# morrislab/rnascan

Measured on AMD Instinct MI355X. Metric: scored windows/sec (seq+struct, w=12), higher is better.
Workload: dtype f64

## Files before the change

include/pfmscan.h:

```cpp
#ifndef PFMSCAN_H
#define PFMSCAN_H

#include <stdint.h>

#ifdef __cplusplus
extern "C" {
#endif

#define PFMSCAN_ABI_VERSION 8
#define PFMSCAN_NCODE   8
#define PFMSCAN_SEP     7
#define PFMSCAN_NSTRUCT 7
#define PFMSCAN_MAX_M   64
#define PFMSCAN_MAX_WIDTH 4096

#define PFMSCAN_OK          0
#define PFMSCAN_E_BADARG   -1
#define PFMSCAN_E_BADSHAPE -2
#define PFMSCAN_E_OOM      -3
#define PFMSCAN_E_HIP      -4
#define PFMSCAN_E_CAPACITY -5

#define PFMSCAN_PROFILE_NONE 0
#define PFMSCAN_PROFILE_F32  1
// ... 138 lines not shown
                                     double *d_hit_struct, uint64_t *d_hit_count, void *stream);
int pfmscan_library_hits_letters_host(pfmscan_ctx *ctx, pfmscan_library *lib,
                                      const uint8_t *codes, const uint8_t *codes2, int64_t n_pos,
                                      const double *thr_seq, const double *thr_struct, int64_t capacity,
                                      int64_t *hit_pos, int32_t *hit_motif, float *hit_seq,
                                      double *hit_struct, int64_t *n_hits);

int pfmscan_debug_credit_table(const double *letter_table, int m, double thr_seq, int bits,
                               uint16_t *credits, double *slack);

int pfmscan_debug_quad_table(const double *letter_table, int m, double thr_seq, uint16_t *credits, double *slack);
int pfmscan_debug_library8_credits(const double *letter_table, int m, double thr, uint16_t *credits, double *slack);

int pfmscan_debug_credit8_table(const double *letter_table, int m, double thr, uint16_t *credits, int *mode);

#define PFMSCAN_UPLOAD_RUNTIME 0
#define PFMSCAN_UPLOAD_STAGED  1
int pfmscan_set_upload_mode(pfmscan_ctx *ctx, int mode);
int pfmscan_upload_source_file(pfmscan_ctx *ctx, const void *base, size_t length, const char *path, int64_t file_offset);
int pfmscan_upload_source_file_checked(pfmscan_ctx *ctx, const void *base, size_t length, const char *path,
                                       int64_t file_offset, int64_t st_dev, int64_t st_ino, int64_t st_size);

int pfmscan_count_bytes(const uint8_t *buf, int64_t n, int64_t *counts , int n_threads);
int pfmscan_fasta_lone_cr(const uint8_t *buf, int64_t n, int *found, int n_threads);
int pfmscan_fasta_index(const uint8_t *buf, int64_t n, int64_t capacity, int64_t *hdr_off,
                        int64_t *hdr_len, int64_t *seq_off, int64_t *seq_end, int64_t *n_letters,
                        int64_t *n_records, int n_threads);
int pfmscan_fasta_ids(const uint8_t *buf, const int64_t *hdr_off, const int64_t *hdr_len,
                      int64_t n_records, int64_t *id_off, int64_t *id_len, int *all_ascii);
int pfmscan_gather_spans(const uint8_t *buf, const int64_t *spans, int64_t n_spans, int separator,
// ... 52 lines not shown
```

rnascan_amd/_lib.py:

```python
import ctypes
import importlib.util
import os
import sys

import numpy as np

HERE = os.path.dirname(os.path.abspath(__file__))
LIB_PATH = os.environ.get("PFMSCAN_LIB") or os.path.join(HERE, "libpfmscan.so")

OK = 0
E_BADARG, E_BADSHAPE, E_OOM, E_HIP, E_CAPACITY = -1, -2, -3, -4, -5
PROFILE_NONE, PROFILE_F32, PROFILE_F64 = 0, 1, 2
SEP = 7
NCODE = 8
NSTRUCT = 7
MAX_M = 64
MAX_WIDTH = 4096
ABI_VERSION = 8

SYMBOLS = [
    "pfmscan_abi_version", "pfmscan_ctx_create", "pfmscan_ctx_destroy", "pfmscan_last_error",
    "pfmscan_device_info", "pfmscan_synchronize", "pfmscan_motif_create", "pfmscan_motif_destroy",
    "pfmscan_pwm_calculate", "pfmscan_scan_dev", "pfmscan_scan_letters_f64_dev", "pfmscan_hits_dev",
    "pfmscan_scan_host", "pfmscan_scan_letters_f64_host", "pfmscan_hits_host", "pfmscan_time_scan_dev",
    "pfmscan_stage", "pfmscan_scan_staged", "pfmscan_hits_staged", "pfmscan_hits_adaptive_dev",
    "pfmscan_library_create", "pfmscan_library_destroy", "pfmscan_library_info", "pfmscan_library_hits_dev",
    "pfmscan_library_hits_staged", "pfmscan_library_hits_host", "pfmscan_library_hits_pipeline_host", "pfmscan_debug_credit_table",
    "pfmscan_library_create_letters", "pfmscan_library_hits_letters_dev", "pfmscan_library_hits_letters_host", "pfmscan_debug_library8_credits",
    "pfmscan_debug_quad_table", "pfmscan_debug_credit8_table",
    "pfmscan_hits_pipeline_host", "pfmscan_staged_positions",
    "pfmscan_hits_letters_f64_dev", "pfmscan_hits_letters_f64_staged", "pfmscan_hits_letters_f64_host",
    "pfmscan_hits_pair_dev", "pfmscan_stage_codes2", "pfmscan_hits_pair_staged", "pfmscan_hits_pair_host", "pfmscan_round_decimals",
    "pfmscan_set_upload_mode", "pfmscan_upload_source_file", "pfmscan_upload_source_file_checked", "pfmscan_fasta_lone_cr", "pfmscan_count_bytes", "pfmscan_fasta_index", "pfmscan_fasta_ids", "pfmscan_gather_spans", "pfmscan_fasta_encode", "pfmscan_tsv_format", "pfmscan_profile_parse", "pfmscan_tsv_number",
    "pfmscan_place_alloc", "pfmscan_place_free", "pfmscan_place_note", "pfmscan_place_trim",
]
TSV_CONST, TSV_I64, TSV_F32, TSV_F64, TSV_INDEXED, TSV_FIXED, TSV_WINDOW, TSV_SPAN = range(8)


class TsvColumn(ctypes.Structure):
    _fields_ = [("kind", ctypes.c_int32), ("reserved", ctypes.c_int32), ("data", ctypes.c_void_p),
                ("aux", ctypes.c_void_p), ("blob", ctypes.c_void_p), ("width", ctypes.c_int64)]



# ... 60 lines not shown
    L.pfmscan_library_create_letters.argtypes = [vp, vp, vp, i32, i32, ctypes.POINTER(vp)]
    L.pfmscan_library_hits_letters_dev.argtypes = [vp, vp, vp, vp, i64, vp, vp, i64, vp, vp, vp, vp, vp, vp]
    L.pfmscan_library_hits_letters_host.argtypes = [vp, vp, vp, vp, i64, vp, vp, i64, vp, vp, vp, vp, ctypes.POINTER(i64)]
    L.pfmscan_library_destroy.argtypes = [vp]
    L.pfmscan_library_destroy.restype = None
    L.pfmscan_library_info.argtypes = [vp, ctypes.POINTER(i32), ctypes.POINTER(i32), ctypes.POINTER(i32), ctypes.POINTER(i32),
                                       ctypes.POINTER(dbl)]
    L.pfmscan_library_hits_dev.argtypes = [vp, vp, vp, vp, i32, i64, vp, vp, i64, vp, vp, vp, vp, vp, vp]
    L.pfmscan_library_hits_staged.argtypes = [vp, vp, vp, vp, i64, vp, vp, vp, vp, ctypes.POINTER(i64)]
    L.pfmscan_library_hits_host.argtypes = [vp, vp, vp, vp, i32, i64, vp, vp, i64, vp, vp, vp, vp, ctypes.POINTER(i64)]
    L.pfmscan_hits_pipeline_host.argtypes = [vp, vp, vp, vp, i32, i64, i64, dbl, dbl, i64, vp, vp, vp, ctypes.POINTER(i64)]
    L.pfmscan_library_hits_pipeline_host.argtypes = [vp, vp, vp, vp, i32, i64, i64, vp, vp, i64, vp, vp, vp, vp, ctypes.POINTER(i64)]
    L.pfmscan_debug_credit_table.argtypes = [vp, i32, dbl, i32, vp, ctypes.POINTER(dbl)]
    L.pfmscan_debug_quad_table.argtypes = [vp, i32, dbl, vp, ctypes.POINTER(dbl)]
    L.pfmscan_debug_credit8_table.argtypes = [vp, i32, dbl, vp, ctypes.POINTER(i32)]
    L.pfmscan_set_upload_mode.argtypes = [vp, i32]
    L.pfmscan_upload_source_file.argtypes = [vp, vp, ctypes.c_size_t, ctypes.c_char_p, i64]
    L.pfmscan_upload_source_file_checked.argtypes = [vp, vp, ctypes.c_size_t, ctypes.c_char_p, i64, i64, i64, i64]
    L.pfmscan_fasta_lone_cr.argtypes = [vp, i64, ctypes.POINTER(i32), i32]
    L.pfmscan_count_bytes.argtypes = [vp, i64, vp, i32]
    L.pfmscan_place_alloc.argtypes = [vp, i32, vp, vp, i32]
    L.pfmscan_place_free.argtypes = [vp, vp]
    L.pfmscan_place_trim.argtypes = [vp]
    L.pfmscan_place_note.argtypes = [vp]
    L.pfmscan_place_note.restype = ctypes.c_char_p
    L.pfmscan_fasta_index.argtypes = [vp, i64, i64, vp, vp, vp, vp, vp, ctypes.POINTER(i64), i32]
    L.pfmscan_fasta_ids.argtypes = [vp, vp, vp, i64, vp, vp, ctypes.POINTER(i32)]
    L.pfmscan_gather_spans.argtypes = [vp, vp, i64, i32, vp, i64, ctypes.POINTER(i64)]
    L.pfmscan_fasta_encode.argtypes = [vp, vp, vp, vp, i64, i64, vp, i32, vp, vp, i32]
    L.pfmscan_profile_parse.argtypes = [ctypes.c_char_p, i64, i32, i64, vp, ctypes.POINTER(i64)]
# ... 712 lines not shown
        if self.has_letters:
            ts = np.ascontiguousarray(np.broadcast_to(np.asarray(thr_seq, dtype=np.float64), (self.n,)))
        tt = None
        if self.has_struct:
            tt = np.ascontiguousarray(np.broadcast_to(np.asarray(-np.inf if thr_struct is None else thr_struct,
                                                                 dtype=np.float64), (self.n,)))
        return ts, tt

    def info(self):
        n, m, npass, per, eps = ctypes.c_int(), ctypes.c_int(), ctypes.c_int(), ctypes.c_int(), ctypes.c_double()
        self._ctx._check(self._L.pfmscan_library_info(self._h, ctypes.byref(n), ctypes.byref(m), ctypes.byref(npass),
                                                      ctypes.byref(per), ctypes.byref(eps)))
        return {"n_motifs": n.value, "m": m.value, "passes": npass.value, "motifs_per_pass": per.value,
                "max_prefilter_eps": eps.value}

    def close(self):
        if getattr(self, "_h", None) and getattr(self._ctx, "_h", None):
            self._L.pfmscan_library_destroy(self._h)
        self._h = None

    def __del__(self):
        try:
            self.close()
        except Exception:
            pass


def credit_table(letter_table, thr_seq, bits=16):
    L = load()
    T = np.ascontiguousarray(letter_table, dtype=np.float64)
    if T.ndim != 2 or T.shape[1] != NCODE:
        raise ValueError("letter_table must be [m][8]")
    m = T.shape[0]
    out = np.zeros(((m + 1) // 2, 16), dtype=np.uint16)
    slack = ctypes.c_double(0.0)
    rc = L.pfmscan_debug_credit_table(_ptr(T), m, float(thr_seq), int(bits), _ptr(out), ctypes.byref(slack))
    if rc != OK:
        raise ValueError("pfmscan_debug_credit_table: bad argument")
    return out, slack.value


def quad_table(letter_table, thr_seq):
    L = load()
    T = np.ascontiguousarray(letter_table, dtype=np.float64)
    if T.ndim != 2 or T.shape[1] != NCODE:
        raise ValueError("letter_table must be [m][8]")
    m = T.shape[0]
    out = np.zeros(((m + 3) // 4, 256), dtype=np.uint16)
    slack = ctypes.c_double(0.0)
    rc = L.pfmscan_debug_quad_table(_ptr(T), m, float(thr_seq), _ptr(out), ctypes.byref(slack))
    if rc != OK:
        raise ValueError("pfmscan_debug_quad_table: bad argument")
    return out, slack.value

# ... 55 lines not shown
```

rnascan_amd/build.py:

```python
import os
import re
import shutil
import subprocess
import sys
import tempfile
from concurrent.futures import ThreadPoolExecutor

HERE = os.path.dirname(os.path.abspath(__file__))
CSRC = os.path.join(HERE, "csrc")
OBJ = os.path.join(CSRC, "_obj")
LIB = os.path.join(HERE, "libpfmscan.so")
SOURCES = ["pfmscan_kernels.hip", "pfmscan_letters8.hip", "pfmscan_letters_fixed.hip", "pfmscan_api.hip", "pfmscan_sort.hip", "pfmscan_library.hip", "pfmscan_library_api.hip", "pfmscan_proflib.hip", "pfmscan_profile_fixed.hip", "pfmscan_place.hip",
           "pfmscan_pipeline.hip", "pfmscan_ingest.hip", "pfmscan_upload.hip"]
HEADERS = ["pfmscan_internal.hpp", "pfmscan_ctx.hpp", "pfmscan_device.hpp", "pfmscan_profile.hpp", "pfmscan_exact.hpp", os.path.join("..", "..", "include", "pfmscan.h")]
DEPS = SOURCES + HEADERS
FLAGS = ["-O3", "--offload-arch=gfx950", "-std=c++17", "-fPIC", "-fno-fast-math", "-Wall"]


def hipcc_path():
    for cand in (os.environ.get("HIPCC"), shutil.which("hipcc"), "/opt/rocm/bin/hipcc"):
        if cand and os.path.exists(cand):
            return cand
    raise RuntimeError("hipcc not found (set HIPCC or install ROCm under /opt/rocm)")


def stale():
    if not os.path.exists(LIB):
# ... 80 lines not shown
```

rnascan_amd/csrc/pfmscan_internal.hpp:

```cpp
#pragma once
#include <hip/hip_runtime.h>
#include <stdint.h>
#include <atomic>
#include "../../include/pfmscan.h"

namespace pfmscan {

struct CredCache {
    double thr = __builtin_nan("");
    int mode = 0;
    uint16_t cr[16 * 16];
};

struct Cred8Cache {
    double thr = __builtin_nan("");
    int mode = 0;
    uint16_t cr[32 * 8];
};

struct QuadSlot {
    double thr = __builtin_nan("");
    uint32_t *d_tab = nullptr;
    uint32_t *h_tab = nullptr;
    hipEvent_t ready = nullptr, used = nullptr;
// ... 169 lines not shown
    const void *profile;
    int profile_dtype;
    int64_t n_pos;
    const double *pssm;
    const double *thr;
    double struct_band;
    const int32_t *finite;
    int n_motifs, m, motif_base;
    int64_t pos_offset;
    int64_t shard_cap;
    int hit_shards;
    int64_t *hit_pos;
    int32_t *hit_motif;
    double *hit_struct;
    unsigned long long *hit_count;
};
hipError_t launch_profile_library(const ProfLibArgs &a, hipStream_t stream);
int64_t profile_library_tile();

hipError_t sort_temp_bytes(int64_t total, int key_bits, size_t *bytes);
hipError_t launch_gather_sorted(const GatherArgs &g, hipStream_t stream);

}
```

rnascan_amd/csrc/pfmscan_library_api.hip:

```cpp
#include <algorithm>
#include <cmath>
#include <cstdlib>
#include <cstring>
#include <new>
#include <string>
#include <vector>

#include "pfmscan_ctx.hpp"

using namespace pfmscan;

namespace {

struct LibPass {
    int motif_base = 0, n_real = 0, nmp = 0, ng = 0;
    int ng_real = 0;
    size_t pairs_off = 0;
    size_t letters_off = 0;
    size_t pssm_off = 0;
    size_t thr_off = 0;
};

}

// ... 56 lines not shown
                out[t * 16 + (c0 | c1 << 2)] = T[(2 * t) * 8 + c0] + (2 * t + 1 < m ? T[(2 * t + 1) * 8 + c1] : 0.0);
}

void pfmscan::quad_sums(const double *T, int m, double *out)
{
    const int nq = (m + 3) / 4;
    for (int t = 0; t < nq; ++t)
        for (int idx = 0; idx < 256; ++idx) {
            double v = 0.0;
            for (int i = 0; i < 4; ++i)
                if (4 * t + i < m) v += T[(4 * t + i) * 8 + ((idx >> (2 * i)) & 3)];
            out[t * 256 + idx] = v;
        }
}

struct pfmscan_library {
    pfmscan_ctx *ctx = nullptr;
    int n = 0, m = 0, npair = 0, np_bucket = 8;
    bool has_struct = false;
    bool has_letters = true;
    bool pair = false;
    bool letters8 = false;
    std::vector<double> rows8;
    double *d_pssm_rows = nullptr;
    int32_t *d_finite = nullptr;
    bool all_finite = false;
    double struct_band = 0.0;
    std::vector<double> pairsum;
    std::vector<LibPass> passes;
    uint16_t *d_pairs = nullptr;
    double *d_letters = nullptr, *d_pssm = nullptr, *d_thr = nullptr;
    size_t pairs_elems = 0, thr_elems = 0;
    std::vector<uint16_t> h_pairs;
    std::vector<double> h_thr;
    std::vector<double> cur_seq, cur_struct, eps;
    bool thr_valid = false;
};

static int lib_fail(pfmscan_ctx *ctx, int code, const std::string &msg) { return fail(ctx, code, msg); }

extern "C" {

// ... 18 lines not shown
        lib->has_struct = true;
        lib->has_letters = false;
        for (int k = 0; k < n_motifs; ++k) lib->struct_band = std::max(lib->struct_band, struct_band(struct_pssms + (size_t)k * m * 7, m));
        std::vector<int32_t> fin((size_t)n_motifs, 1);
        for (int k = 0; k < n_motifs; ++k)
            for (int i = 0; i < m * 7; ++i)
                if (!std::isfinite(struct_pssms[(size_t)k * m * 7 + i])) fin[(size_t)k] = 0;
        if (std::getenv("PFMSCAN_FORCE_GENERIC")) std::fill(fin.begin(), fin.end(), 0);
        const size_t cells = (size_t)n_motifs * m * 7;
        hipError_t e = hipMalloc((void **)&lib->d_pssm_rows, cells * 8);
        if (e == hipSuccess) e = hipMemcpy(lib->d_pssm_rows, struct_pssms, cells * 8, hipMemcpyHostToDevice);
        if (e == hipSuccess) e = hipMalloc((void **)&lib->d_finite, (size_t)n_motifs * 4);
        if (e == hipSuccess) e = hipMemcpy(lib->d_finite, fin.data(), (size_t)n_motifs * 4, hipMemcpyHostToDevice);
        if (e == hipSuccess) e = hipMalloc((void **)&lib->d_thr, (size_t)n_motifs * 8);
        lib->thr_elems = (size_t)n_motifs;
        if (e != hipSuccess) {
            pfmscan_library_destroy(lib);
            return fail_hip(ctx, e, "uploading the library tables");
        }
        *out = lib;
        return PFMSCAN_OK;
    }
    return create_seq_library(ctx, letter_tables, struct_pssms, 7, n_motifs, m, out);
}

}

static int create_seq_library(pfmscan_ctx *ctx, const double *letter_tables, const double *struct_pssms, int ncol, int n_motifs, int m,
                              pfmscan_library **out)
{
// ... 160 lines not shown
            return lib_fail(ctx, PFMSCAN_E_BADSHAPE, "column 7 of every letter table must be NaN (the foreign code)");
    if (seq_tables) return create_seq_library(ctx, seq_tables, struct_tables, 8, n_motifs, m, out);
    return create_letters8_library(ctx, struct_tables, n_motifs, m, out);
}

void pfmscan_library_destroy(pfmscan_library *lib)
{
    if (!lib) return;
    if (lib->ctx) (void)hipSetDevice(lib->ctx->device);
    if (lib->d_pairs) (void)hipFree(lib->d_pairs);
    if (lib->d_letters) (void)hipFree(lib->d_letters);
    if (lib->d_pssm) (void)hipFree(lib->d_pssm);
    if (lib->d_thr) (void)hipFree(lib->d_thr);
    if (lib->d_pssm_rows) (void)hipFree(lib->d_pssm_rows);
    if (lib->d_finite) (void)hipFree(lib->d_finite);
    delete lib;
}

int pfmscan_debug_credit_table(const double *letter_table, int m, double thr_seq, int bits, uint16_t *credits, double *slack)
{
    if (!letter_table || !credits || m < 1 || m > PFMSCAN_MAX_M || std::isnan(thr_seq)) return PFMSCAN_E_BADARG;
    if (bits == 0) bits = lib_credit_bits(lib_np_bucket(m));
    if (bits != 10 && bits != 16) return PFMSCAN_E_BADARG;
    const int npair = (m + 1) / 2;
    std::vector<double> ps((size_t)npair * 16);
    pair_sums(letter_table, m, ps.data());
    const double s = build_credits(ps.data(), npair, thr_seq, credits, bits);
    if (slack) *slack = s;
    return PFMSCAN_OK;
}

// ... 38 lines not shown

}

static int lib_set_thresholds(pfmscan_ctx *ctx, pfmscan_library *lib, const double *thr_seq, const double *thr_struct, hipStream_t st)
{
    const int n = lib->n, npair = lib->npair;
    if (!lib->has_letters && !lib->letters8) {
        for (int k = 0; k < n; ++k)
            if (std::isnan(thr_struct[k])) return lib_fail(ctx, PFMSCAN_E_BADARG, "NaN threshold");
        if (lib->thr_valid && std::equal(thr_struct, thr_struct + n, lib->cur_struct.begin())) return PFMSCAN_OK;
        HIP_TRY(ctx, hipStreamSynchronize(st));
        lib->h_thr.assign(thr_struct, thr_struct + n);
        HIP_TRY(ctx, hipMemcpyAsync(lib->d_thr, lib->h_thr.data(), (size_t)n * 8, hipMemcpyHostToDevice, st));
        lib->cur_struct.assign(thr_struct, thr_struct + n);
        lib->eps.assign((size_t)n, 0.0);
        lib->thr_valid = true;
        return PFMSCAN_OK;
    }
    if (lib->letters8) {
        const int rows = lib->npair;
        for (int k = 0; k < n; ++k) {
            if (std::isnan(thr_struct[k])) return lib_fail(ctx, PFMSCAN_E_BADARG, "NaN threshold");
            if (thr_struct[k] == -INFINITY)
                return lib_fail(ctx, PFMSCAN_E_BADARG, "library hits need a finite threshold (every window would be a hit; use the all-scores entry points)");
        }
        if (lib->thr_valid && std::equal(thr_struct, thr_struct + n, lib->cur_struct.begin())) return PFMSCAN_OK;
        HIP_TRY(ctx, hipStreamSynchronize(st));
        lib->thr_valid = false;
        lib->h_pairs.assign(lib->pairs_elems, (uint16_t)0);
        lib->h_thr.assign(lib->thr_elems, 0.0);
// ... 130 lines not shown
        a.n_pos = n_pos;
        a.pssm = lib->d_pssm_rows;
        a.thr = lib->d_thr;
        a.struct_band = lib->struct_band;
        a.finite = lib->d_finite;
        a.n_motifs = lib->n;
        a.m = lib->m;
        a.motif_base = 0;
        a.pos_offset = pos_offset;
        a.shard_cap = sink.shard_cap;
        a.hit_shards = sink.shards;
        a.hit_pos = sink.pos;
        a.hit_motif = sink.motif;
        a.hit_struct = sink.st;
        a.hit_count = sink.count;
        hipError_t e = launch_profile_library(a, st);
        if (e != hipSuccess) return fail_hip(ctx, e, "launch k_profile_lib");
        return PFMSCAN_OK;
    }
    const LibPass &first_pass = lib->passes[0];
    bool teams = lib->has_struct && !lib->pair && lib->passes.size() > 1 && n_pos >= (int64_t)8 * ctx->n_cu * LIB_SEG &&
                 ctx->n_cu >= 16 && !std::getenv("PFMSCAN_LIB_SEQUENTIAL");
    for (const LibPass &ps : lib->passes) teams = teams && ps.ng == first_pass.ng;
    const int64_t max_span = (int64_t)1 << 31;
    for (int64_t base = 0; base < n_pos; base += max_span) {
        const int64_t span_segs = (std::min<int64_t>(max_span, n_pos - base) + LIB_SEG - 1) / LIB_SEG;
        const size_t per_launch = teams && span_segs >= ctx->n_cu ? 4 : 1;
        for (size_t p0 = 0; p0 < lib->passes.size(); p0 += per_launch) {
            const LibPass &ps = lib->passes[p0];
            const size_t nt = std::min(per_launch, lib->passes.size() - p0);
// ... 411 lines not shown
```

rnascan_amd/csrc/pfmscan_proflib.hip:

```cpp
#include <float.h>
#include <math.h>

#include "pfmscan_internal.hpp"
#include "pfmscan_exact.hpp"

namespace pfmscan {

constexpr int PL_LANES = 256;
constexpr int PL_GROUPS = 4;
constexpr int PL_BLOCK = PL_LANES * PL_GROUPS;
#ifndef PL_V_OVERRIDE
#define PL_V_OVERRIDE 5
#endif
constexpr int PL_V = PL_V_OVERRIDE;
constexpr int PL_NS = PL_V + 1;
constexpr int PL_UNROLL = (PL_NS % 2) ? 2 * PL_NS : PL_NS;
constexpr int PL_TILE = PL_LANES * PL_V;
#ifndef PL_WAIT_FIRST
#define PL_WAIT_FIRST 1
#endif
#ifndef PL_STAGGER
#define PL_STAGGER 0
#endif
#ifndef PL_INTERLEAVE
#define PL_INTERLEAVE 0
#endif
constexpr int PL_QCAP = 128;

typedef uint32_t pl_u32x4 __attribute__((ext_vector_type(4)));
typedef double pl_f64x2 __attribute__((ext_vector_type(2)));

__device__ __forceinline__ double pl_nan_to_num(double d)
{
    double c = fmin(fmax(d, -DBL_MAX), DBL_MAX);
    return (d != d) ? 0.0 : c;
}

__host__ __device__ constexpr int pl_tile_vals(int m) { return ((PL_TILE + m) * 7 + 3) / 4 * 4; }
__host__ __device__ constexpr int pl_tile_bytes(int m) { return pl_tile_vals(m) * 8; }
__host__ __device__ constexpr int pl_queue_bytes() { return (PL_BLOCK / 64) * PL_QCAP * (8 + 4); }

__device__ __forceinline__ double pl_window_slow(const double *tile, int local, const double *__restrict__ pssm, int m)
{
    double score = 0.0;
#pragma unroll 1
    for (int j = 0; j < m; ++j) {
        const double *r = tile + (local + j) * 7;
        double d = r[0] * pssm[j * 7];
#pragma unroll 1
        for (int k = 1; k < 7; ++k) d = fma(r[k], pssm[j * 7 + k], d);
        score += pl_nan_to_num(d);
    }
    return score;
}

template <bool FINITE>
__device__ __forceinline__ void pl_score_motif(const double *tile, const double *__restrict__ pssm, const double *__restrict__ pssm_next,
                                               int m, int la, double (&acc)[PL_V], double (&P)[7])
{
    constexpr int V = PL_V, NS = PL_NS;
    const volatile __attribute__((address_space(3))) double *vt = (const volatile __attribute__((address_space(3))) double *)tile;
    double rows[NS][7];
#pragma unroll
    for (int s = 0; s < V; ++s) {
#pragma unroll
        for (int k = 0; k < 7; ++k) rows[s][k] = vt[(la + s) * 7 + k];
        acc[s] = 0.0;
    }
#if defined(PL_ABLATE) && (PL_ABLATE & 2)
// ... 46 lines not shown
    for (; j0 + PL_UNROLL <= m; j0 += PL_UNROLL) {
#pragma unroll
        for (int uu = 0; uu < PL_UNROLL; ++uu) step(uu, j0 + uu);
    }
#pragma unroll
    for (int uu = 0; uu < PL_UNROLL - 1; ++uu) {
        if (j0 + uu < m) step(uu, j0 + uu);
    }
    if (m & 1) {
#pragma unroll
        for (int k = 0; k < 7; ++k) P[k] = Q[k];
    }
    if (FINITE) {
#pragma unroll
        for (int v = 0; v < V; ++v)
            if (!(fabs(acc[v]) <= DBL_MAX)) acc[v] = pl_window_slow(tile, la + v, pssm, m);
    }
}

template <typename PROF_T>
__global__ __launch_bounds__(PL_BLOCK) void k_profile_lib(const ProfLibArgs a)
{
    constexpr int V = PL_V;
    constexpr int PER = 16 / (int)sizeof(PROF_T);
    typedef PROF_T vec_t __attribute__((ext_vector_type(PER)));
    extern __shared__ __align__(16) unsigned char smem[];
    const int m = a.m;
    double *tile = reinterpret_cast<double *>(smem);
    const int lane = threadIdx.x & 63;
    const int wave = __builtin_amdgcn_readfirstlane(threadIdx.x >> 6);
    const int group = wave / (PL_LANES / 64);
// ... 120 lines not shown
                }
            }
        }
        k = kn;
        if (kn < nm) kn = (int)__builtin_amdgcn_readfirstlane(draw());
    }
    if (qn > 0) flush();
}

int64_t profile_library_tile() { return PL_TILE; }

hipError_t launch_profile_library(const ProfLibArgs &a, hipStream_t stream)
{
    if (a.n_pos <= 0 || a.n_motifs <= 0) return hipSuccess;
    if (a.n_motifs > 65536 || a.m < 1 || a.m > PFMSCAN_MAX_M) return hipErrorInvalidValue;
    const unsigned grid = (unsigned)((a.n_pos + PL_TILE - 1) / PL_TILE);
    const size_t lds = (size_t)pl_tile_bytes(a.m) + pl_queue_bytes() + 16;
    static std::atomic<uint64_t> done_f{0}, done_d{0};
    if (a.profile_dtype == PFMSCAN_PROFILE_F64) {
        hipError_t e = allow_dynamic_lds(reinterpret_cast<const void *>(k_profile_lib<double>), done_d, 160 * 1024);
        if (e != hipSuccess) return e;
        hipLaunchKernelGGL(k_profile_lib<double>, dim3(grid), dim3(PL_BLOCK), lds, stream, a);
    } else {
        hipError_t e = allow_dynamic_lds(reinterpret_cast<const void *>(k_profile_lib<float>), done_f, 160 * 1024);
        if (e != hipSuccess) return e;
        hipLaunchKernelGGL(k_profile_lib<float>, dim3(grid), dim3(PL_BLOCK), lds, stream, a);
    }
    return hipGetLastError();
}

// ... 2 lines not shown
```

Baseline: 144.9 billion.

## Add MFMA f16 prefilter for structure-profile library scan with exact f64 verify

```diff
diff --git a/include/pfmscan.h b/include/pfmscan.h
--- a/include/pfmscan.h
+++ b/include/pfmscan.h
@@ -176,6 +176,10 @@
 
 int pfmscan_debug_credit8_table(const double *letter_table, int m, double thr, uint16_t *credits, int *mode);
 
+int pfmscan_debug_proflib_bound(const double *pssm, int m, double thr, double band, float R, uint16_t *bfrag, double *coef,
+                                float *thr_eff, int *eligible);
+int pfmscan_library_proflib_stats(pfmscan_library *lib, long long *mfma_runs, long long *valu_runs, long long *survivors);
+
 #define PFMSCAN_UPLOAD_RUNTIME 0
 #define PFMSCAN_UPLOAD_STAGED  1
 int pfmscan_set_upload_mode(pfmscan_ctx *ctx, int mode);
diff --git a/rnascan_amd/_lib.py b/rnascan_amd/_lib.py
--- a/rnascan_amd/_lib.py
+++ b/rnascan_amd/_lib.py
@@ -27,7 +27,7 @@
     "pfmscan_library_create", "pfmscan_library_destroy", "pfmscan_library_info", "pfmscan_library_hits_dev",
     "pfmscan_library_hits_staged", "pfmscan_library_hits_host", "pfmscan_library_hits_pipeline_host", "pfmscan_debug_credit_table",
     "pfmscan_library_create_letters", "pfmscan_library_hits_letters_dev", "pfmscan_library_hits_letters_host", "pfmscan_debug_library8_credits",
-    "pfmscan_debug_quad_table", "pfmscan_debug_credit8_table",
+    "pfmscan_debug_quad_table", "pfmscan_debug_credit8_table", "pfmscan_debug_proflib_bound", "pfmscan_library_proflib_stats",
     "pfmscan_hits_pipeline_host", "pfmscan_staged_positions",
     "pfmscan_hits_letters_f64_dev", "pfmscan_hits_letters_f64_staged", "pfmscan_hits_letters_f64_host",
     "pfmscan_hits_pair_dev", "pfmscan_stage_codes2", "pfmscan_hits_pair_staged", "pfmscan_hits_pair_host", "pfmscan_round_decimals",
@@ -118,6 +118,10 @@
     L.pfmscan_debug_credit_table.argtypes = [vp, i32, dbl, i32, vp, ctypes.POINTER(dbl)]
     L.pfmscan_debug_quad_table.argtypes = [vp, i32, dbl, vp, ctypes.POINTER(dbl)]
     L.pfmscan_debug_credit8_table.argtypes = [vp, i32, dbl, vp, ctypes.POINTER(i32)]
+    L.pfmscan_debug_proflib_bound.argtypes = [vp, i32, dbl, dbl, ctypes.c_float, vp, vp, ctypes.POINTER(ctypes.c_float),
+                                              ctypes.POINTER(i32)]
+    L.pfmscan_library_proflib_stats.argtypes = [vp, ctypes.POINTER(ctypes.c_longlong), ctypes.POINTER(ctypes.c_longlong),
+                                                ctypes.POINTER(ctypes.c_longlong)]
     L.pfmscan_set_upload_mode.argtypes = [vp, i32]
     L.pfmscan_upload_source_file.argtypes = [vp, vp, ctypes.c_size_t, ctypes.c_char_p, i64]
     L.pfmscan_upload_source_file_checked.argtypes = [vp, vp, ctypes.c_size_t, ctypes.c_char_p, i64, i64, i64, i64]
@@ -860,6 +864,11 @@
         return {"n_motifs": n.value, "m": m.value, "passes": npass.value, "motifs_per_pass": per.value,
                 "max_prefilter_eps": eps.value}
 
+    def proflib_stats(self):
+        a, b, c = ctypes.c_longlong(), ctypes.c_longlong(), ctypes.c_longlong()
+        self._ctx._check(self._L.pfmscan_library_proflib_stats(self._h, ctypes.byref(a), ctypes.byref(b), ctypes.byref(c)))
+        return {"mfma_runs": a.value, "valu_runs": b.value, "survivors": c.value}
+
     def close(self):
         if getattr(self, "_h", None) and getattr(self._ctx, "_h", None):
             self._L.pfmscan_library_destroy(self._h)
@@ -884,6 +893,23 @@
     if rc != OK:
         raise ValueError("pfmscan_debug_credit_table: bad argument")
     return out, slack.value
+
+
+def proflib_bound(pssm, thr, band, R=1.0):
+    L = load()
+    P = np.ascontiguousarray(pssm, dtype=np.float64)
+    if P.ndim != 2 or P.shape[1] != NSTRUCT:
+        raise ValueError("pssm must be [m][7]")
+    m = P.shape[0]
+    b = np.zeros((2 * ((m + 1) // 2), 8), dtype=np.uint16)
+    coef = np.zeros(4, dtype=np.float64)
+    te, el = ctypes.c_float(0.0), ctypes.c_int(0)
+    rc = L.pfmscan_debug_proflib_bound(_ptr(P), m, float(thr), float(band), float(R), _ptr(b) if m <= 32 else None,
+                                       _ptr(coef), ctypes.byref(te), ctypes.byref(el))
+    if rc != OK:
+        raise ValueError("pfmscan_debug_proflib_bound: bad argument")
+    return {"b": b, "A": coef[0], "E": coef[1], "c0": coef[2], "c1": coef[3], "thr_eff": te.value,
+            "eligible": bool(el.value & 1), "ninf": bool(el.value & 2)}
 
 
 def quad_table(letter_table, thr_seq):
diff --git a/rnascan_amd/build.py b/rnascan_amd/build.py
--- a/rnascan_amd/build.py
+++ b/rnascan_amd/build.py
@@ -10,7 +10,7 @@
 CSRC = os.path.join(HERE, "csrc")
 OBJ = os.path.join(CSRC, "_obj")
 LIB = os.path.join(HERE, "libpfmscan.so")
-SOURCES = ["pfmscan_kernels.hip", "pfmscan_letters8.hip", "pfmscan_letters_fixed.hip", "pfmscan_api.hip", "pfmscan_sort.hip", "pfmscan_library.hip", "pfmscan_library_api.hip", "pfmscan_proflib.hip", "pfmscan_profile_fixed.hip", "pfmscan_place.hip",
+SOURCES = ["pfmscan_kernels.hip", "pfmscan_letters8.hip", "pfmscan_letters_fixed.hip", "pfmscan_api.hip", "pfmscan_sort.hip", "pfmscan_library.hip", "pfmscan_library_api.hip", "pfmscan_proflib.hip", "pfmscan_proflib_mfma.hip", "pfmscan_profile_fixed.hip", "pfmscan_place.hip",
            "pfmscan_pipeline.hip", "pfmscan_ingest.hip", "pfmscan_upload.hip"]
 HEADERS = ["pfmscan_internal.hpp", "pfmscan_ctx.hpp", "pfmscan_device.hpp", "pfmscan_profile.hpp", "pfmscan_exact.hpp", os.path.join("..", "..", "include", "pfmscan.h")]
 DEPS = SOURCES + HEADERS
diff --git a/rnascan_amd/csrc/pfmscan_internal.hpp b/rnascan_amd/csrc/pfmscan_internal.hpp
--- a/rnascan_amd/csrc/pfmscan_internal.hpp
+++ b/rnascan_amd/csrc/pfmscan_internal.hpp
@@ -207,8 +207,15 @@
     int32_t *hit_motif;
     double *hit_struct;
     unsigned long long *hit_count;
+    const void *bfrag;
+    const double *slack_c0, *slack_c1;
+    const int32_t *ninf;
+    int n_pairs;
+    unsigned long long *survivors;
 };
 hipError_t launch_profile_library(const ProfLibArgs &a, hipStream_t stream);
+hipError_t launch_profile_library_mfma(const ProfLibArgs &a, hipStream_t stream);
+constexpr int PROFLIB_MFMA_MAX_M = 32;
 int64_t profile_library_tile();
 
 hipError_t sort_temp_bytes(int64_t total, int key_bits, size_t *bytes);
diff --git a/rnascan_amd/csrc/pfmscan_library_api.hip b/rnascan_amd/csrc/pfmscan_library_api.hip
--- a/rnascan_amd/csrc/pfmscan_library_api.hip
+++ b/rnascan_amd/csrc/pfmscan_library_api.hip
@@ -94,6 +94,63 @@
         }
 }
 
+constexpr double PROFLIB_CELL_MAX = 60000.0;
+
+struct ProflibBound {
+    double A = 0.0, E = 0.0, c0 = 0.0, c1 = 0.0;
+    bool ninf = false;
+    bool ok = false;
+};
+
+static inline double gamma_n(double n, double u) { return n * u / (1.0 - n * u); }
+
+static ProflibBound proflib_bound(const double *pssm, int m, uint16_t *bfrag)
+{
+    ProflibBound b;
+    const int S = (m + 1) / 2;
+    if (bfrag) std::fill(bfrag, bfrag + (size_t)2 * S * 8, (uint16_t)0);
+    b.ok = m >= 1 && m <= PROFLIB_MFMA_MAX_M;
+    for (int j = 0; j < m; ++j) {
+        bool row_ninf = false;
+        for (int k = 0; k < 7; ++k) {
+            const double v = pssm[j * 7 + k];
+            if (v == -INFINITY) row_ninf = true;
+            else if (!std::isfinite(v) || std::fabs(v) > PROFLIB_CELL_MAX) b.ok = false;
+        }
+        b.ninf = b.ninf || row_ninf;
+        if (row_ninf || !b.ok) continue;
+        double ma = 0.0, me = 0.0;
+        for (int k = 0; k < 7; ++k) {
+            const double v = pssm[j * 7 + k];
+            const _Float16 h = (_Float16)v;
+            const double hv = (double)h;
+            ma = std::max(ma, std::fabs(hv));
+            me = std::max(me, std::fabs(v - hv));
+            if (bfrag) std::memcpy(bfrag + (size_t)j * 8 + k, &h, 2);
+        }
+        b.A += ma;
+        b.E += me;
+    }
+    if (!b.ok) return b;
+    const double K = 17.0 * S + 1.0;
+    const double g32 = gamma_n(K, 0x1p-23), g64 = gamma_n(8.0 * m, 0x1p-52);
+    const double delta = 7.0 * m * 0x1p-24;
+    const double up = 1.0 + 0x1p-20;
+    b.c1 = (b.A * 0x1p-10 + b.E + g32 * b.A * (1.0 + 0x1p-10) + g64 * (b.A + b.E)) * up;
+    b.c0 = (delta * b.A * (1.0 + g32)) * up;
+    return b;
+}
+
+static float proflib_thr_eff(double t, double band, double c0, double c1, float R)
+{
+    const double slack = c0 + c1 * (double)R;
+    const double x = (t - band) - slack - (std::fabs(t) + band + slack) * 0x1p-40;
+    float f = (float)x;
+    if (std::isnan(x)) return f;
+    if ((double)f > x) f = std::nextafter(f, -INFINITY);
+    return f;
+}
+
 struct pfmscan_library {
     pfmscan_ctx *ctx = nullptr;
     int n = 0, m = 0, npair = 0, np_bucket = 8;
@@ -106,6 +163,12 @@
     int32_t *d_finite = nullptr;
     bool all_finite = false;
     double struct_band = 0.0;
+    bool mfma_cells = false, thr_all_finite = false;
+    void *d_bfrag = nullptr;
+    double *d_slack = nullptr;
+    int32_t *d_ninf = nullptr;
+    unsigned long long *d_survivors = nullptr;
+    long long runs_mfma = 0, runs_valu = 0;
     std::vector<double> pairsum;
     std::vector<LibPass> passes;
     uint16_t *d_pairs = nullptr;
@@ -154,6 +217,32 @@
         if (e == hipSuccess) e = hipMemcpy(lib->d_finite, fin.data(), (size_t)n_motifs * 4, hipMemcpyHostToDevice);
         if (e == hipSuccess) e = hipMalloc((void **)&lib->d_thr, (size_t)n_motifs * 8);
         lib->thr_elems = (size_t)n_motifs;
+        if (e == hipSuccess && m <= PROFLIB_MFMA_MAX_M) {
+            const int S = (m + 1) / 2, npairs = (n_motifs + 63) / 64;
+            const size_t per = (size_t)2 * S * 8;
+            std::vector<uint16_t> bf((size_t)npairs * 64 * per, (uint16_t)0);
+            std::vector<double> slack((size_t)2 * n_motifs);
+            std::vector<int32_t> ninf((size_t)n_motifs);
+            bool ok = true;
+            for (int k = 0; k < n_motifs && ok; ++k) {
+                const ProflibBound b = proflib_bound(struct_pssms + (size_t)k * m * 7, m, bf.data() + (size_t)k * per);
+                ok = b.ok;
+                slack[(size_t)k] = b.c0;
+                slack[(size_t)n_motifs + k] = b.c1;
+                ninf[(size_t)k] = b.ninf ? 1 : 0;
+            }
+            if (ok) {
+                e = hipMalloc(&lib->d_bfrag, bf.size() * 2);
+                if (e == hipSuccess) e = hipMemcpy(lib->d_bfrag, bf.data(), bf.size() * 2, hipMemcpyHostToDevice);
+                if (e == hipSuccess) e = hipMalloc((void **)&lib->d_slack, slack.size() * 8);
+                if (e == hipSuccess) e = hipMemcpy(lib->d_slack, slack.data(), slack.size() * 8, hipMemcpyHostToDevice);
+                if (e == hipSuccess) e = hipMalloc((void **)&lib->d_ninf, ninf.size() * 4);
+                if (e == hipSuccess) e = hipMemcpy(lib->d_ninf, ninf.data(), ninf.size() * 4, hipMemcpyHostToDevice);
+                if (e == hipSuccess) e = hipMalloc((void **)&lib->d_survivors, 8);
+                if (e == hipSuccess) e = hipMemset(lib->d_survivors, 0, 8);
+                lib->mfma_cells = e == hipSuccess;
+            }
+        }
         if (e != hipSuccess) {
             pfmscan_library_destroy(lib);
             return fail_hip(ctx, e, "uploading the library tables");
@@ -344,7 +433,50 @@
     if (lib->d_thr) (void)hipFree(lib->d_thr);
     if (lib->d_pssm_rows) (void)hipFree(lib->d_pssm_rows);
     if (lib->d_finite) (void)hipFree(lib->d_finite);
+    if (lib->d_bfrag) (void)hipFree(lib->d_bfrag);
+    if (lib->d_slack) (void)hipFree(lib->d_slack);
+    if (lib->d_ninf) (void)hipFree(lib->d_ninf);
+    if (lib->d_survivors) (void)hipFree(lib->d_survivors);
     delete lib;
+}
+
+int pfmscan_library_proflib_stats(pfmscan_library *lib, long long *mfma_runs, long long *valu_runs, long long *survivors)
+{
+    if (!lib) return PFMSCAN_E_BADARG;
+    if (mfma_runs) *mfma_runs = lib->runs_mfma;
+    if (valu_runs) *valu_runs = lib->runs_valu;
+    if (survivors) {
+        unsigned long long v = 0;
+        if (lib->d_survivors) {
+            HIP_TRY(lib->ctx, hipSetDevice(lib->ctx->device));
+            HIP_TRY(lib->ctx, hipDeviceSynchronize());
+            HIP_TRY(lib->ctx, hipMemcpy(&v, lib->d_survivors, 8, hipMemcpyDeviceToHost));
+        }
+        *survivors = (long long)v;
+    }
+    return PFMSCAN_OK;
+}
+
+int pfmscan_debug_proflib_bound(const double *pssm, int m, double thr, double band, float R, uint16_t *bfrag, double *coef,
+                                float *thr_eff, int *eligible)
+{
+    if (!pssm || m < 1 || m > PFMSCAN_MAX_M || std::isnan(thr) || !(band >= 0.0)) return PFMSCAN_E_BADARG;
+    std::vector<uint16_t> tmp;
+    if (!bfrag && m <= PROFLIB_MFMA_MAX_M) {
+        tmp.resize((size_t)2 * ((m + 1) / 2) * 8);
+        bfrag = tmp.data();
+    }
+    const ProflibBound b = proflib_bound(pssm, m, m <= PROFLIB_MFMA_MAX_M ? bfrag : nullptr);
+    if (coef) {
+        coef[0] = b.A;
+        coef[1] = b.E;
+        coef[2] = b.c0;
+        coef[3] = b.c1;
+    }
+    const bool ok = b.ok && std::isfinite(thr);
+    if (thr_eff) *thr_eff = ok ? proflib_thr_eff(thr, band, b.c0, b.c1, R) : NAN;
+    if (eligible) *eligible = (ok ? 1 : 0) | (b.ninf ? 2 : 0);
+    return PFMSCAN_OK;
 }
 
 int pfmscan_debug_credit_table(const double *letter_table, int m, double thr_seq, int bits, uint16_t *credits, double *slack)
@@ -413,6 +545,7 @@
         HIP_TRY(ctx, hipMemcpyAsync(lib->d_thr, lib->h_thr.data(), (size_t)n * 8, hipMemcpyHostToDevice, st));
         lib->cur_struct.assign(thr_struct, thr_struct + n);
         lib->eps.assign((size_t)n, 0.0);
+        lib->thr_all_finite = std::all_of(thr_struct, thr_struct + n, [](double t) { return std::isfinite(t); });
         lib->thr_valid = true;
         return PFMSCAN_OK;
     }
@@ -573,6 +706,19 @@
         a.hit_motif = sink.motif;
         a.hit_struct = sink.st;
         a.hit_count = sink.count;
+        const char *valu_env = std::getenv("PFMSCAN_PROFLIB_VALU");
+        const bool valu = valu_env && std::atoi(valu_env) != 0;
+        if (lib->mfma_cells && lib->thr_all_finite && !valu) {
+            a.bfrag = lib->d_bfrag;
+            a.slack_c0 = lib->d_slack;
+            a.slack_c1 = lib->d_slack + lib->n;
+            a.ninf = lib->d_ninf;
+            a.n_pairs = (lib->n + 63) / 64;
+            a.survivors = lib->d_survivors;
+            ++lib->runs_mfma;
+        } else {
+            ++lib->runs_valu;
+        }
         hipError_t e = launch_profile_library(a, st);
         if (e != hipSuccess) return fail_hip(ctx, e, "launch k_profile_lib");
         return PFMSCAN_OK;
diff --git a/rnascan_amd/csrc/pfmscan_proflib.hip b/rnascan_amd/csrc/pfmscan_proflib.hip
--- a/rnascan_amd/csrc/pfmscan_proflib.hip
+++ b/rnascan_amd/csrc/pfmscan_proflib.hip
@@ -3,6 +3,7 @@
 
 #include "pfmscan_internal.hpp"
 #include "pfmscan_exact.hpp"
+#include "pfmscan_proflib.hpp"
 
 namespace pfmscan {
 
@@ -30,29 +31,9 @@
 typedef uint32_t pl_u32x4 __attribute__((ext_vector_type(4)));
 typedef double pl_f64x2 __attribute__((ext_vector_type(2)));
 
-__device__ __forceinline__ double pl_nan_to_num(double d)
-{
-    double c = fmin(fmax(d, -DBL_MAX), DBL_MAX);
-    return (d != d) ? 0.0 : c;
-}
-
 __host__ __device__ constexpr int pl_tile_vals(int m) { return ((PL_TILE + m) * 7 + 3) / 4 * 4; }
 __host__ __device__ constexpr int pl_tile_bytes(int m) { return pl_tile_vals(m) * 8; }
 __host__ __device__ constexpr int pl_queue_bytes() { return (PL_BLOCK / 64) * PL_QCAP * (8 + 4); }
-
-__device__ __forceinline__ double pl_window_slow(const double *tile, int local, const double *__restrict__ pssm, int m)
-{
-    double score = 0.0;
-#pragma unroll 1
-    for (int j = 0; j < m; ++j) {
-        const double *r = tile + (local + j) * 7;
-        double d = r[0] * pssm[j * 7];
-#pragma unroll 1
-        for (int k = 1; k < 7; ++k) d = fma(r[k], pssm[j * 7 + k], d);
-        score += pl_nan_to_num(d);
-    }
-    return score;
-}
 
 template <bool FINITE>
 __device__ __forceinline__ void pl_score_motif(const double *tile, const double *__restrict__ pssm, const double *__restrict__ pssm_next,
@@ -129,7 +110,7 @@
     if (FINITE) {
 #pragma unroll
         for (int v = 0; v < V; ++v)
-            if (!(fabs(acc[v]) <= DBL_MAX)) acc[v] = pl_window_slow(tile, la + v, pssm, m);
+            if (!(fabs(acc[v]) <= DBL_MAX)) acc[v] = pl_window_slow(tile + (la + v) * 7, pssm, m);
     }
 }
 
@@ -280,6 +261,7 @@
 {
     if (a.n_pos <= 0 || a.n_motifs <= 0) return hipSuccess;
     if (a.n_motifs > 65536 || a.m < 1 || a.m > PFMSCAN_MAX_M) return hipErrorInvalidValue;
+    if (a.bfrag) return launch_profile_library_mfma(a, stream);
     const unsigned grid = (unsigned)((a.n_pos + PL_TILE - 1) / PL_TILE);
     const size_t lds = (size_t)pl_tile_bytes(a.m) + pl_queue_bytes() + 16;
     static std::atomic<uint64_t> done_f{0}, done_d{0};
diff --git a/rnascan_amd/csrc/pfmscan_proflib.hpp b/rnascan_amd/csrc/pfmscan_proflib.hpp
--- /dev/null
+++ b/rnascan_amd/csrc/pfmscan_proflib.hpp
@@ -0,0 +1,64 @@
+#pragma once
+#include <float.h>
+#include <math.h>
+#include <hip/hip_runtime.h>
+
+#include "pfmscan_exact.hpp"
+
+namespace pfmscan {
+
+__device__ __forceinline__ double pl_nan_to_num(double d)
+{
+    double c = fmin(fmax(d, -DBL_MAX), DBL_MAX);
+    return (d != d) ? 0.0 : c;
+}
+
+template <typename ROW_T>
+__device__ __forceinline__ double pl_window_slow(const ROW_T *rows, const double *__restrict__ pssm, int m)
+{
+    double score = 0.0;
+#pragma unroll 1
+    for (int j = 0; j < m; ++j) {
+        const ROW_T *r = rows + j * 7;
+        double d = (double)r[0] * pssm[j * 7];
+#pragma unroll 1
+        for (int k = 1; k < 7; ++k) d = fma((double)r[k], pssm[j * 7 + k], d);
+        score += pl_nan_to_num(d);
+    }
+    return score;
+}
+
+template <bool FINITE, typename ROW_T>
+__device__ __forceinline__ double pl_window_fast(const ROW_T *rows, const double *__restrict__ pssm, int m)
+{
+    double acc = 0.0;
+    if (FINITE) {
+#pragma unroll 1
+        for (int j = 0; j < m; ++j)
+#pragma unroll
+            for (int k = 0; k < 7; ++k) acc = fma((double)rows[j * 7 + k], pssm[j * 7 + k], acc);
+        if (!(fabs(acc) <= DBL_MAX)) acc = pl_window_slow(rows, pssm, m);
+    } else {
+#pragma unroll 1
+        for (int j = 0; j < m; ++j) {
+            double d = (double)rows[j * 7] * pssm[j * 7];
+#pragma unroll
+            for (int k = 1; k < 7; ++k) d = fma((double)rows[j * 7 + k], pssm[j * 7 + k], d);
+            acc += pl_nan_to_num(d);
+        }
+    }
+    return acc;
+}
+
+template <typename ROW_T>
+__device__ __forceinline__ bool pl_decide(double &acc, double t, double band, const ROW_T *rows, const double *__restrict__ pssm, int m)
+{
+    if (!(acc > t - band)) return false;
+    if (acc <= t + band) {
+        acc = struct_window_rounded(rows, m, [&](int j, int c) { return pssm[j * 7 + c]; });
+        return acc > t;
+    }
+    return true;
+}
+
+}
diff --git a/rnascan_amd/csrc/pfmscan_proflib_mfma.hip b/rnascan_amd/csrc/pfmscan_proflib_mfma.hip
--- /dev/null
+++ b/rnascan_amd/csrc/pfmscan_proflib_mfma.hip
@@ -0,0 +1,271 @@
+#include <float.h>
+#include <math.h>
+
+#include "pfmscan_internal.hpp"
+#include "pfmscan_exact.hpp"
+#include "pfmscan_proflib.hpp"
+
+namespace pfmscan {
+
+constexpr int PM_BLOCK = 256;
+constexpr int PM_WAVES = PM_BLOCK / 64;
+constexpr int PM_TILE = 1024;
+constexpr int PM_NB = PM_TILE / 32;
+constexpr int PM_ROWS = PM_TILE + 32;
+constexpr int PM_SQCAP = 128;
+constexpr int PM_HQCAP = 128;
+constexpr float PM_RMAX = 32768.0f;
+
+typedef _Float16 pm_h8 __attribute__((ext_vector_type(8)));
+typedef float pm_f16 __attribute__((ext_vector_type(16)));
+
+__device__ __forceinline__ float pm_thr(const ProfLibArgs &a, int q, float R, uint32_t flags)
+{
+    if ((flags & 1u) || ((flags & 2u) && a.ninf[q])) return __builtin_nanf("");
+    const double t = a.thr[q], band = a.struct_band;
+    const double slack = a.slack_c0[q] + a.slack_c1[q] * (double)R;
+    const double x = (t - band) - slack - (fabs(t) + band + slack) * 0x1p-40;
+    return __double2float_rd(x);
+}
+
+template <typename PROF_T, int S>
+__global__ __launch_bounds__(PM_BLOCK) void k_profile_lib_mfma(const ProfLibArgs a)
+{
+    __shared__ pm_h8 rows[PM_ROWS];
+    __shared__ uint32_t sq[PM_WAVES][PM_SQCAP];
+    __shared__ double hq_sc[PM_WAVES][PM_HQCAP];
+    __shared__ uint32_t hq_wm[PM_WAVES][PM_HQCAP];
+    __shared__ float red_r[PM_WAVES];
+    __shared__ uint32_t red_f[PM_WAVES];
+
+    const int m = a.m;
+    const int lane = threadIdx.x & 63;
+    const int wave = __builtin_amdgcn_readfirstlane(threadIdx.x >> 6);
+    const int64_t n_pos = a.n_pos;
+    const int64_t tile0 = (int64_t)blockIdx.x * PM_TILE;
+    const PROF_T *__restrict__ prof = reinterpret_cast<const PROF_T *>(a.profile);
+
+    float rmax = 0.0f;
+    uint32_t flags = 0;
+    for (int r = threadIdx.x; r < PM_TILE + 2 * S - 1; r += PM_BLOCK) {
+        const int64_t p = tile0 + r;
+        double f[7];
+        if (p < n_pos) {
+            const PROF_T *src = prof + p * 7;
+#pragma unroll
+            for (int k = 0; k < 7; ++k) f[k] = (double)__builtin_nontemporal_load(src + k);
+        } else {
+#pragma unroll
+            for (int k = 0; k < 7; ++k) f[k] = 0.0;
+        }
+        double s = 0.0;
+        bool neg = false;
+        pm_h8 h;
+#pragma unroll
+        for (int k = 0; k < 7; ++k) {
+            s += fabs(f[k]);
+            neg = neg || f[k] < 0.0;
+            h[k] = (_Float16)(float)f[k];
+        }
+        h[7] = (_Float16)0.0f;
+        rows[r] = h;
+        if (!(s <= (double)PM_RMAX)) flags |= 1u;
+        else rmax = fmaxf(rmax, __double2float_ru(s * (1.0 + 0x1p-48)));
+        if (neg) flags |= 2u;
+    }
+#pragma unroll
+    for (int o = 32; o > 0; o >>= 1) rmax = fmaxf(rmax, __shfl_xor(rmax, o));
+    const uint32_t fw = (__builtin_amdgcn_ballot_w64((flags & 1u) != 0) ? 1u : 0u) | (__builtin_amdgcn_ballot_w64((flags & 2u) != 0) ? 2u : 0u);
+    if (lane == 0) {
+        red_r[wave] = rmax;
+        red_f[wave] = fw;
+    }
+    __syncthreads();
+    float R = red_r[0];
+    uint32_t tflags = red_f[0];
+#pragma unroll
+    for (int w = 1; w < PM_WAVES; ++w) {
+        R = fmaxf(R, red_r[w]);
+        tflags |= red_f[w];
+    }
+
+    const int shard = blockIdx.x & (a.hit_shards - 1);
+    unsigned long long *counter = a.hit_count + (size_t)shard * HIT_COUNTER_STRIDE;
+    const unsigned long long shard_off = (unsigned long long)shard * (unsigned long long)a.shard_cap;
+    auto wave_sync = [&]() {
+        __builtin_amdgcn_fence(__ATOMIC_RELEASE, "wavefront");
+        __builtin_amdgcn_wave_barrier();
+        __builtin_amdgcn_fence(__ATOMIC_ACQUIRE, "wavefront");
+    };
+    int hn = 0;
+    auto flush = [&]() {
+        wave_sync();
+        unsigned long long base = 0;
+        if (lane == 0) base = atomicAdd(counter, (unsigned long long)hn);
+        const uint32_t lo = __builtin_amdgcn_readfirstlane((uint32_t)base), hi = __builtin_amdgcn_readfirstlane((uint32_t)(base >> 32));
+        base = ((unsigned long long)hi << 32) | lo;
+        for (int i = lane; i < hn; i += 64) {
+            const unsigned long long slot = base + (unsigned long long)i;
+            if ((int64_t)slot < a.shard_cap) {
+                const uint32_t wm = hq_wm[wave][i];
+                a.hit_pos[shard_off + slot] = tile0 + (int64_t)(wm >> 16) + a.pos_offset;
+                a.hit_motif[shard_off + slot] = a.motif_base + (int32_t)(wm & 0xFFFFu);
+                a.hit_struct[shard_off + slot] = hq_sc[wave][i];
+            }
+        }
+        wave_sync();
+        hn = 0;
+    };
+    int qn = 0;
+    auto verify = [&]() {
+        wave_sync();
+        for (int i0 = 0; i0 < qn; i0 += 64) {
+            const int i = i0 + lane;
+            bool pass = false;
+            double sc = 0.0;
+            uint32_t e = 0;
+            if (i < qn) {
+                e = sq[wave][i];
+                const int q = (int)(e & 0xFFFFu);
+                const PROF_T *rw = prof + (tile0 + (int64_t)(e >> 16)) * 7;
+                const double *ps = a.pssm + (size_t)q * m * 7;
+                sc = a.finite[q] ? pl_window_fast<true>(rw, ps, m) : pl_window_fast<false>(rw, ps, m);
+                pass = pl_decide(sc, a.thr[q], a.struct_band, rw, ps, m);
+            }
+            const unsigned long long mk = __builtin_amdgcn_ballot_w64(pass);
+            if (mk) {
+                if (hn + 64 > PM_HQCAP) flush();
+                if (pass) {
+                    const int slot = hn + (int)__builtin_amdgcn_mbcnt_hi((uint32_t)(mk >> 32), __builtin_amdgcn_mbcnt_lo((uint32_t)mk, 0u));
+                    hq_sc[wave][slot] = sc;
+                    hq_wm[wave][slot] = e;
+                }
+                hn += __popcll(mk);
+            }
+        }
+        if (lane == 0 && a.survivors) atomicAdd(a.survivors, (unsigned long long)qn);
+        wave_sync();
+        qn = 0;
+    };
+
+    const int64_t live_all = n_pos - m + 1 - tile0;
+    const int live_n = live_all < 0 ? 0 : (live_all > PM_TILE ? PM_TILE : (int)live_all);
+    const int nm = a.n_motifs;
+    const int npairs = a.n_pairs;
+    const int nch = npairs >= PM_WAVES ? 1 : (PM_WAVES + npairs - 1) / npairs;
+    const int items = npairs * nch;
+    const pm_h8 *__restrict__ bfrag = reinterpret_cast<const pm_h8 *>(a.bfrag);
+    const int col = lane & 31, half = lane >> 5;
+#pragma unroll 1
+    for (int it = wave; it < items; it += PM_WAVES) {
+        const int pr = it / nch, ch = it - pr * nch;
+        const int b_lo = ch * PM_NB / nch, b_hi = (ch + 1) * PM_NB / nch;
+        const int q0 = pr * 64 + col, q1 = q0 + 32;
+        pm_h8 B0[S], B1[S];
+#pragma unroll
+        for (int s = 0; s < S; ++s) {
+            B0[s] = bfrag[(size_t)q0 * (2 * S) + 2 * s + half];
+            B1[s] = bfrag[(size_t)q1 * (2 * S) + 2 * s + half];
+        }
+        const bool ok0 = q0 < nm, ok1 = q1 < nm;
+        const float th0 = ok0 ? pm_thr(a, q0, R, tflags) : 0.0f;
+        const float th1 = ok1 ? pm_thr(a, q1, R, tflags) : 0.0f;
+#pragma unroll 1
+        for (int b = b_lo; b < b_hi; ++b) {
+            if (b * 32 >= live_n) break;
+            pm_f16 c0 = {}, c1 = {};
+            const pm_h8 *ar = rows + b * 32 + col + half;
+#pragma unroll
+            for (int s = 0; s < S; ++s) {
+                const pm_h8 av = ar[2 * s];
+                c0 = __builtin_amdgcn_mfma_f32_32x32x16_f16(av, B0[s], c0, 0, 0, 0);
+                c1 = __builtin_amdgcn_mfma_f32_32x32x16_f16(av, B1[s], c1, 0, 0, 0);
+            }
+            const int lim = __builtin_amdgcn_readfirstlane(live_n - b * 32) - 4 * half;
+            auto keep = [&](int g, int r) -> bool {
+                const float v = g ? c1[r] : c0[r];
+                const bool ok = g ? ok1 : ok0;
+                const float th = g ? th1 : th0;
+                return ok && ((r & 3) + 8 * (r >> 2) < lim) && !(v <= th);
+            };
+            bool any = false;
+            if (lim >= 32) {
+                bool a0 = false, a1 = false;
+#pragma unroll
+                for (int r = 0; r < 16; ++r) {
+                    a0 |= !(c0[r] <= th0);
+                    a1 |= !(c1[r] <= th1);
+                }
+                any = (a0 & ok0) | (a1 & ok1);
+            } else {
+#pragma unroll
+                for (int r = 0; r < 16; ++r) {
+                    any |= keep(0, r);
+                    any |= keep(1, r);
+                }
+            }
+            if (__builtin_expect(__builtin_amdgcn_ballot_w64(any) == 0, 1)) continue;
+#pragma unroll
+            for (int g = 0; g < 2; ++g) {
+#pragma unroll
+                for (int r = 0; r < 16; ++r) {
+                    const bool p = keep(g, r);
+                    const unsigned long long mk = __builtin_amdgcn_ballot_w64(p);
+                    if (!mk) continue;
+                    if (qn + 64 > PM_SQCAP) verify();
+                    if (p) {
+                        const int slot = qn + (int)__builtin_amdgcn_mbcnt_hi((uint32_t)(mk >> 32), __builtin_amdgcn_mbcnt_lo((uint32_t)mk, 0u));
+                        const uint32_t w = (uint32_t)(b * 32 + (r & 3) + 8 * (r >> 2) + 4 * half);
+                        sq[wave][slot] = (w << 16) | (uint32_t)(g ? q1 : q0);
+                    }
+                    qn += __popcll(mk);
+                }
+            }
+        }
+    }
+    if (qn > 0) verify();
+    if (hn > 0) flush();
+}
+
+template <typename PROF_T, int S>
+static hipError_t pm_launch(const ProfLibArgs &a, hipStream_t stream)
+{
+    const unsigned grid = (unsigned)((a.n_pos + PM_TILE - 1) / PM_TILE);
+    hipLaunchKernelGGL((k_profile_lib_mfma<PROF_T, S>), dim3(grid), dim3(PM_BLOCK), 0, stream, a);
+    return hipGetLastError();
+}
+
+template <typename PROF_T>
+static hipError_t pm_launch_dtype(const ProfLibArgs &a, hipStream_t stream)
+{
+    switch ((a.m + 1) / 2) {
+    case 1: return pm_launch<PROF_T, 1>(a, stream);
+    case 2: return pm_launch<PROF_T, 2>(a, stream);
+    case 3: return pm_launch<PROF_T, 3>(a, stream);
+    case 4: return pm_launch<PROF_T, 4>(a, stream);
+    case 5: return pm_launch<PROF_T, 5>(a, stream);
+    case 6: return pm_launch<PROF_T, 6>(a, stream);
+    case 7: return pm_launch<PROF_T, 7>(a, stream);
+    case 8: return pm_launch<PROF_T, 8>(a, stream);
+    case 9: return pm_launch<PROF_T, 9>(a, stream);
+    case 10: return pm_launch<PROF_T, 10>(a, stream);
+    case 11: return pm_launch<PROF_T, 11>(a, stream);
+    case 12: return pm_launch<PROF_T, 12>(a, stream);
+    case 13: return pm_launch<PROF_T, 13>(a, stream);
+    case 14: return pm_launch<PROF_T, 14>(a, stream);
+    case 15: return pm_launch<PROF_T, 15>(a, stream);
+    case 16: return pm_launch<PROF_T, 16>(a, stream);
+    default: return hipErrorInvalidValue;
+    }
+}
+
+hipError_t launch_profile_library_mfma(const ProfLibArgs &a, hipStream_t stream)
+{
+    if (a.n_pos <= 0 || a.n_motifs <= 0) return hipSuccess;
+    if (a.n_motifs > 65535 || a.m < 1 || a.m > PROFLIB_MFMA_MAX_M || !a.bfrag || !a.slack_c0 || !a.slack_c1 || !a.ninf ||
+        a.n_pairs != (a.n_motifs + 63) / 64)
+        return hipErrorInvalidValue;
+    return a.profile_dtype == PFMSCAN_PROFILE_F64 ? pm_launch_dtype<double>(a, stream) : pm_launch_dtype<float>(a, stream);
+}
+
+}
```

After: 144.8 billion (median of 6 runs). No clear change (-0.1%).
